# facebook/winterfell

Hardware: NVIDIA H100
Metric: prover_ms (lower is better)
Workload: dtype u64

## Files before the change

### winterfell_b200/csrc/minidft.cuh

```cuda
#pragma once
#include "gl64.cuh"

__device__ __forceinline__ void bf2(u64& a, u64& b) { gl_butterfly(a, b); }
template <int R>
__device__ __forceinline__ void mini_dft(u64* x);
template <>
__device__ __forceinline__ void mini_dft<1>(u64* x) { bf2(x[0], x[1]); }
template <>
__device__ __forceinline__ void mini_dft<2>(u64* x) {
    bf2(x[0], x[2]);
    bf2(x[1], x[3]);
    x[3] = gl_mul_2exp<48>(x[3]);
    bf2(x[0], x[1]);
    bf2(x[2], x[3]);
}
template <>
__device__ __forceinline__ void mini_dft<3>(u64* x);
template <>
__device__ __forceinline__ void mini_dft<3>(u64* x) {
    bf2(x[0], x[4]);
    bf2(x[1], x[5]);
    bf2(x[2], x[6]);
    bf2(x[3], x[7]);
    x[5] = gl_mul_2exp<24>(x[5]);
    x[6] = gl_mul_2exp<48>(x[6]);
    x[7] = gl_mul_2exp<72>(x[7]);
    mini_dft<2>(x);
    mini_dft<2>(x + 4);
}
template <>
__device__ __forceinline__ void mini_dft<4>(u64* x) {
    bf2(x[0], x[8]);
    bf2(x[1], x[9]);
    bf2(x[2], x[10]);
    bf2(x[3], x[11]);
    bf2(x[4], x[12]);
    bf2(x[5], x[13]);
    bf2(x[6], x[14]);
    bf2(x[7], x[15]);
    x[9] = gl_mul_2exp<12>(x[9]);
    x[10] = gl_mul_2exp<24>(x[10]);
    x[11] = gl_mul_2exp<36>(x[11]);
    x[12] = gl_mul_2exp<48>(x[12]);
    x[13] = gl_mul_2exp<60>(x[13]);
    x[14] = gl_mul_2exp<72>(x[14]);
    x[15] = gl_mul_2exp<84>(x[15]);
    mini_dft<3>(x);
    mini_dft<3>(x + 8);
}
template <>
__device__ __forceinline__ void mini_dft<5>(u64* x) {
#pragma unroll
    for (int q = 0; q < 16; q++) bf2(x[q], x[q + 16]);
    x[17] = gl_mul_2exp<6>(x[17]);
    x[18] = gl_mul_2exp<12>(x[18]);
    x[19] = gl_mul_2exp<18>(x[19]);
    x[20] = gl_mul_2exp<24>(x[20]);
    x[21] = gl_mul_2exp<30>(x[21]);
    x[22] = gl_mul_2exp<36>(x[22]);
    x[23] = gl_mul_2exp<42>(x[23]);
    x[24] = gl_mul_2exp<48>(x[24]);
    x[25] = gl_mul_2exp<54>(x[25]);
    x[26] = gl_mul_2exp<60>(x[26]);
    x[27] = gl_mul_2exp<66>(x[27]);
    x[28] = gl_mul_2exp<72>(x[28]);
    x[29] = gl_mul_2exp<78>(x[29]);
    x[30] = gl_mul_2exp<84>(x[30]);
    x[31] = gl_mul_2exp<90>(x[31]);
    mini_dft<4>(x);
    mini_dft<4>(x + 16);
}
__device__ __forceinline__ u32 brev(u32 v, int bits) { return __brev(v) >> (32 - bits); }

__device__ __forceinline__ u64 tw_lookup(const u64* tab, u32 e, u32 half) {
    u64 t = tab[e & (half - 1)];
    return (e & half) ? gl_neg(t) : t;
}
```

### winterfell_b200/csrc/ntt2.cu

```cuda
#include "minidft.cuh"
#include "ntt.cuh"

#ifndef NTT2_THREADS
#define NTT2_THREADS 256
#endif
#ifndef NTT2_MINB
#define NTT2_MINB 2
#endif
#define NTT2_TILE_ELEMS 8192

template <int LOGS>
struct Plan {
    static constexpr int rounds = LOGS >= 9 ? 3 : 2;
    static constexpr int r0 = (LOGS == 8) ? 4 : 3;
    static constexpr int r1 = (LOGS == 11 || LOGS == 8 || LOGS == 7) ? 4 : 3;
    static constexpr int r2 = LOGS >= 9 ? LOGS - r0 - r1 : 0;
    static_assert(LOGS >= 6 && LOGS <= 11, "plan covers 2^6 .. 2^11");
    static_assert(r0 + r1 + r2 == LOGS && (rounds == 2 || (r2 == 3 || r2 == 4)), "radices must add up");
    static constexpr int lanes = LOGS == 11 ? 4 : 8;
    static constexpr int tw0_entries = 1 << LOGS;
    static constexpr int tw1_entries = rounds == 3 ? (1 << (LOGS - r0)) : 0;
    static constexpr int tw_entries = tw0_entries + tw1_entries;
};
template <int LOGS> __host__ __device__ constexpr int plan_radix(int k) { return k == 0 ? Plan<LOGS>::r0 : (k == 1 ? Plan<LOGS>::r1 : Plan<LOGS>::r2); }
template <int LOGS> __host__ __device__ constexpr int plan_stage(int k) { return k == 0 ? 0 : (k == 1 ? Plan<LOGS>::r0 : Plan<LOGS>::r0 + Plan<LOGS>::r1); }

template <int LK>
__host__ __device__ constexpr u32 swz_const(u32 r) {
    u32 x = r >> LK, h = 0;
    while (x) { h ^= x & ((1u << LK) - 1); x >>= LK; }
    return h;
}
template <int LK>
__device__ __forceinline__ u32 swz_hash(u32 r) {
    if (LK == 1) return __popc(r >> 1) & 1;
    u32 x = r >> 2;
    x ^= x >> 4;
    x ^= x >> 8;
    x ^= x >> 2;
    return x & 3;
}
template <int LK>
__device__ __forceinline__ u32 prow(u32 r) { return r ^ swz_hash<LK>(r); }

__device__ __forceinline__ void bulk_init(u64* mbar, int tid) {
    if (tid == 0) {
        u32 mb = (u32)__cvta_generic_to_shared(mbar);
        asm volatile("mbarrier.init.shared::cta.b64 [%0], 1;" ::"r"(mb));
        asm volatile("fence.mbarrier_init.release.cluster;" ::: "memory");
    }
}
__device__ __forceinline__ void bulk_expect(u64* mbar, u32 bytes) {
    u32 mb = (u32)__cvta_generic_to_shared(mbar);
    asm volatile("mbarrier.arrive.expect_tx.shared::cta.b64 _, [%0], %1;" ::"r"(mb), "r"(bytes) : "memory");
}
__device__ __forceinline__ void bulk_copy(void* smem_dst, const void* gsrc, u32 bytes, u64* mbar) {
    u32 mb = (u32)__cvta_generic_to_shared(mbar), dst = (u32)__cvta_generic_to_shared(smem_dst);
    asm volatile("cp.async.bulk.shared::cluster.global.mbarrier::complete_tx::bytes [%0], [%1], %2, [%3];" ::"r"(dst), "l"(gsrc), "r"(bytes),
                 "r"(mb)
                 : "memory");
}
__device__ __forceinline__ void bulk_wait(u64* mbar) {
    u32 mb = (u32)__cvta_generic_to_shared(mbar), done = 0;
    while (!done)
        asm volatile("{\n\t.reg .pred p;\n\tmbarrier.try_wait.parity.shared::cta.b64 p, [%1], 0;\n\tselp.u32 %0, 1, 0, p;\n\t}" : "=r"(done) : "r"(mb) : "memory");
}

__device__ __forceinline__ void cp_async16(void* smem_dst, const void* gsrc, bool ok) {
    const u32 dst = (u32)__cvta_generic_to_shared(smem_dst);
    asm volatile("cp.async.cg.shared.global [%0], [%1], 16, %2;" ::"r"(dst), "l"(gsrc), "r"(ok ? 16 : 0) : "memory");
}
__device__ __forceinline__ void cp_async8(void* smem_dst, const void* gsrc, bool ok) {
    const u32 dst = (u32)__cvta_generic_to_shared(smem_dst);
    asm volatile("cp.async.ca.shared.global [%0], [%1], 8, %2;" ::"r"(dst), "l"(gsrc), "r"(ok ? 8 : 0) : "memory");
}
__device__ __forceinline__ void cp_async_commit() { asm volatile("cp.async.commit_group;" ::: "memory"); }
__device__ __forceinline__ void cp_async_wait_all() { asm volatile("cp.async.wait_group 0;" ::: "memory"); }

template <int LOGS, int K>
__device__ __forceinline__ void tile_round(u64* __restrict__ s, const u64* __restrict__ tw, const u64* __restrict__ pre, int tid) {
    constexpr int LANES = Plan<LOGS>::lanes, LK = LANES == 8 ? 1 : 2;
    constexpr int R = plan_radix<LOGS>(K), ST = plan_stage<LOGS>(K);
    constexpr int LOGSPAN = LOGS - ST - R;
    constexpr u32 SPAN = 1u << LOGSPAN;
    constexpr bool LAST = LOGSPAN == 0;
    constexpr u32 TASKS = (1u << LOGS) * LANES / 16;
    if (R == 4) {
        for (u32 task = tid; task < TASKS; task += NTT2_THREADS) {
            const u32 lane = task % LANES, bf = task / LANES;
            const u32 lo = bf & (SPAN - 1), base = ((bf >> LOGSPAN) << (LOGSPAN + 4)) + lo;
            const u32 hb = swz_hash<LK>(base);
            u64 x[16];
#pragma unroll
            for (int q = 0; q < 16; q++) {
                const u32 row = (base + ((u32)q << LOGSPAN)) ^ (hb ^ swz_const<LK>((u32)q << LOGSPAN));
                x[q] = s[row * LANES + lane];
            }
            if (K == 0 && pre) {
#pragma unroll
                for (int q = 0; q < 16; q++) x[q] = gl_mul(x[q], __ldg(pre + base + ((u32)q << LOGSPAN)));
            }
            mini_dft<4>(x);
            if (!LAST) {
                const ulonglong2* t2 = reinterpret_cast<const ulonglong2*>(tw + (size_t)lo * 16);
#pragma unroll
                for (int h = 0; h < 8; h++) {
                    const ulonglong2 w = t2[h];
                    if (h > 0) x[2 * h] = gl_mul(x[2 * h], w.x);
                    x[2 * h + 1] = gl_mul(x[2 * h + 1], w.y);
                }
            }
#pragma unroll
            for (int q = 0; q < 16; q++) {
                const u32 row = (base + ((u32)q << LOGSPAN)) ^ (hb ^ swz_const<LK>((u32)q << LOGSPAN));
                s[row * LANES + lane] = x[q];
            }
        }
    } else {
        constexpr int LP = LANES / 2;
        for (u32 task = tid; task < TASKS; task += NTT2_THREADS) {
            const u32 lp = task % LP, bf = task / LP;
            const u32 lo = bf & (SPAN - 1), base = ((bf >> LOGSPAN) << (LOGSPAN + 3)) + lo;
            const u32 hb = swz_hash<LK>(base);
            u64 xa[8], xb[8];
#pragma unroll
            for (int q = 0; q < 8; q++) {
                const u32 row = (base + ((u32)q << LOGSPAN)) ^ (hb ^ swz_const<LK>((u32)q << LOGSPAN));
                const ulonglong2 v = *reinterpret_cast<const ulonglong2*>(s + row * LANES + 2 * lp);
                xa[q] = v.x;
                xb[q] = v.y;
            }
            if (K == 0 && pre) {
#pragma unroll
                for (int q = 0; q < 8; q++) {
                    const u64 f = __ldg(pre + base + ((u32)q << LOGSPAN));
                    xa[q] = gl_mul(xa[q], f);
                    xb[q] = gl_mul(xb[q], f);
                }
            }
            mini_dft<3>(xa);
            mini_dft<3>(xb);
            if (!LAST) {
                const ulonglong2* t2 = reinterpret_cast<const ulonglong2*>(tw + (size_t)lo * 8);
#pragma unroll
                for (int h = 0; h < 4; h++) {
                    const ulonglong2 w = t2[h];
                    if (h > 0) { xa[2 * h] = gl_mul(xa[2 * h], w.x); xb[2 * h] = gl_mul(xb[2 * h], w.x); }
                    xa[2 * h + 1] = gl_mul(xa[2 * h + 1], w.y);
                    xb[2 * h + 1] = gl_mul(xb[2 * h + 1], w.y);
                }
            }
#pragma unroll
            for (int q = 0; q < 8; q++) {
                const u32 row = (base + ((u32)q << LOGSPAN)) ^ (hb ^ swz_const<LK>((u32)q << LOGSPAN));
                *reinterpret_cast<ulonglong2*>(s + row * LANES + 2 * lp) = make_ulonglong2(xa[q], xb[q]);
            }
        }
    }
}

template <int MODE, int LOGS>
__global__ void __launch_bounds__(NTT2_THREADS, NTT2_MINB) ntt2_pass_kernel(const NttPassParams p) {
    extern __shared__ __align__(16) u64 smem[];
    constexpr int LANES = Plan<LOGS>::lanes, LK = LANES == 8 ? 1 : 2, LP = LANES / 2;
    constexpr u32 S = 1u << LOGS;
    const int tid = threadIdx.x;
    const int W = p.W, logW = 31 - __clz(W);
    const int T = W >= LANES ? 1 : (LANES >> logW);
    const int chunks = W >= LANES ? W / LANES : 1;
    u64* s = smem;
    u64* rtw = s + (size_t)S * LANES;
    u64* ctw = rtw + Plan<LOGS>::tw_entries;
    u64* mbar = ctw + (p.has_post ? (size_t)S * T : 0);

    const bool ymap = p.y_in_out;
    const u32 tc = ymap ? blockIdx.y : blockIdx.x;
    const u32 tile = tc / chunks, q0 = (tc % chunks) * LANES;
    const u32 g = ymap ? blockIdx.z : blockIdx.y, b = ymap ? blockIdx.x : blockIdx.z;
    const u32 R = 1u << p.logR, C = 1u << p.logC;
    const u32 ncols = MODE == NTT_STRIDED ? C : R;

    {
        const u64* in = p.in + (size_t)g * p.in_seg_stride + (size_t)b * p.in_batch_stride;
        const u32 lp = tid % LP;
        const u32 l0 = 2 * lp;
        const u32 t0 = W >= LANES ? 0 : (l0 >> logW), t1 = W >= LANES ? 0 : ((l0 + 1) >> logW);
        const u32 w0 = W >= LANES ? q0 + l0 : (l0 & (W - 1)), w1 = W >= LANES ? q0 + l0 + 1 : ((l0 + 1) & (W - 1));
        const u32 c0 = tile * T + t0, c1 = tile * T + t1;
        const bool ok0 = c0 < ncols, ok1 = c1 < ncols;
        const bool yin = MODE == NTT_CONTIG && ymap;
        const u64 istride = MODE == NTT_STRIDED ? ((u64)W << p.logC) : (yin ? ((u64)p.out_row_mul << p.logR) * p.out_W : (u64)W);
        const u64* a0 = MODE == NTT_STRIDED ? in + (size_t)c0 * W + w0
                        : yin ? in + ((size_t)c0 * p.out_row_mul + (size_t)b * p.out_row_add) * p.out_W + p.out_col0 + w0
                              : in + (((size_t)c0 << p.logC) * W + w0);
        const u64* a1 = MODE == NTT_STRIDED ? in + (size_t)c1 * W + w1
                        : yin ? in + ((size_t)c1 * p.out_row_mul + (size_t)b * p.out_row_add) * p.out_W + p.out_col0 + w1
                              : in + (((size_t)c1 << p.logC) * W + w1);
        if (!ok0) a0 = p.in;
        if (!ok1) a1 = p.in;
        const u64 s0 = ok0 ? istride : 0, s1 = ok1 ? istride : 0;
        const bool vec = p.vec_in;
        constexpr u32 ROWS_PER_IT = NTT2_THREADS / LP;
#pragma unroll 4
        for (u32 i = tid / LP; i < S; i += ROWS_PER_IT) {
            u64* dst = s + prow<LK>(i) * LANES + l0;
            if (vec) {
                cp_async16(dst, a0 + i * s0, ok0);
            } else {
                cp_async8(dst, a0 + i * s0, ok0);
                cp_async8(dst + 1, a1 + i * s1, ok1);
            }
        }
        cp_async_commit();
    }

    bulk_init(mbar, tid);
    __syncthreads();
    if (tid == 0) {
        bulk_expect(mbar, Plan<LOGS>::tw_entries * 8);
        bulk_copy(rtw, p.sub_tw, Plan<LOGS>::tw_entries * 8, mbar);
    }

    if (p.has_post && T == 1) {
        const u32 M = 1u << p.logM, lo_mask = (1u << p.tw_split) - 1, c = tile;
        auto wpow = [&](u64 e64) {
            u32 e = (u32)(e64 & (M - 1));
            if (p.inverse && e) e = M - e;
            return gl_mul(p.tw_hi[e >> p.tw_split], p.tw_lo[e & lo_mask]);
        };
        u64 K = wpow((u64)(p.batch0 + b) * p.b_mul * c);
        if (p.ctab) K = gl_mul(K, p.ctab[c < ncols ? c : 0]);
        if (p.cconst != 1) K = gl_mul(K, p.cconst);
        const u64 step = wpow((u64)NTT2_THREADS * p.a_mul * c);
        u64 x = gl_mul(K, wpow((u64)tid * p.a_mul * c));
        for (u32 j = tid; j < S; j += NTT2_THREADS) {
            ctw[j] = x;
            x = gl_mul(x, step);
        }
    } else if (p.has_post) {
        const u32 M = 1u << p.logM, lo_mask = (1u << p.tw_split) - 1;
        for (u32 idx = tid; idx < S * (u32)T; idx += NTT2_THREADS) {
            const u32 j = idx / T, tt = idx % T, c = tile * T + tt;
            u64 e64 = ((u64)j * p.a_mul + (u64)(p.batch0 + b) * p.b_mul) * c;
            u32 e = (u32)(e64 & (M - 1));
            if (p.inverse && e) e = M - e;
            u64 x = gl_mul(p.tw_hi[e >> p.tw_split], p.tw_lo[e & lo_mask]);
            if (p.ctab) x = gl_mul(x, p.ctab[c < ncols ? c : 0]);
            if (p.cconst != 1) x = gl_mul(x, p.cconst);
            ctw[idx] = x;
        }
    }

    cp_async_wait_all();
    bulk_wait(mbar);
    __syncthreads();

    tile_round<LOGS, 0>(s, rtw, p.pre_tab ? p.pre_tab + (size_t)b * p.pre_batch_stride : nullptr, tid);
    __syncthreads();
    if (Plan<LOGS>::rounds == 3) {
        tile_round<LOGS, 1>(s, rtw + Plan<LOGS>::tw0_entries, nullptr, tid);
        __syncthreads();
        tile_round<LOGS, 2>(s, nullptr, nullptr, tid);
    } else {
        tile_round<LOGS, 1>(s, nullptr, nullptr, tid);
    }
    __syncthreads();

    u64* out = p.out + (size_t)g * p.out_seg_stride + (size_t)b * p.out_batch_stride;
    {
        const u32 lp = tid % LP, l0 = 2 * lp;
        const u32 t0 = W >= LANES ? 0 : (l0 >> logW), t1 = W >= LANES ? 0 : ((l0 + 1) >> logW);
        const u32 w0 = W >= LANES ? q0 + l0 : (l0 & (W - 1)), w1 = W >= LANES ? q0 + l0 + 1 : ((l0 + 1) & (W - 1));
        const u32 c0 = tile * T + t0, c1 = tile * T + t1;
        const bool ok0 = c0 < ncols, ok1 = c1 < ncols;
        u64 *o0, *o1, jstride;
        if (MODE == NTT_STRIDED && ymap) {
            o0 = out + (((size_t)c0 << p.logR) * p.out_row_mul + (size_t)b * p.out_row_add) * p.out_W + p.out_col0 + w0;
            o1 = out + (((size_t)c1 << p.logR) * p.out_row_mul + (size_t)b * p.out_row_add) * p.out_W + p.out_col0 + w1;
            jstride = (u64)p.out_row_mul * p.out_W;
        } else if (MODE == NTT_STRIDED) {
            o0 = out + (size_t)c0 * W + w0;
            o1 = out + (size_t)c1 * W + w1;
            jstride = (u64)W << p.logC;
        } else {
            o0 = out + ((size_t)c0 * p.out_row_mul + (size_t)b * p.out_row_add) * p.out_W + p.out_col0 + w0;
            o1 = out + ((size_t)c1 * p.out_row_mul + (size_t)b * p.out_row_add) * p.out_W + p.out_col0 + w1;
            jstride = ((u64)p.out_row_mul << p.logR) * p.out_W;
        }
        const bool post = p.has_post, scale = !p.has_post && p.cconst != 1, vec = p.vec_out;
        const u32 inv_mask = p.inverse ? (S - 1) : 0;
        constexpr u32 ROWS_PER_IT = NTT2_THREADS / LP;
#pragma unroll 4
        for (u32 j = tid / LP; j < S; j += ROWS_PER_IT) {
            const u32 jf = inv_mask ? ((S - j) & inv_mask) : j;
            const u32 r = __brev(jf) >> (32 - LOGS);
            ulonglong2 v = *reinterpret_cast<const ulonglong2*>(s + prow<LK>(r) * LANES + l0);
            if (post) {
                const u64 f0 = ctw[j * T + t0];
                v.x = gl_mul(v.x, f0);
                v.y = gl_mul(v.y, t1 == t0 ? f0 : ctw[j * T + t1]);
            } else if (scale) {
                v.x = gl_mul(v.x, p.cconst);
                v.y = gl_mul(v.y, p.cconst);
            }
            if (vec) {
                if (ok0) *reinterpret_cast<ulonglong2*>(o0 + (u64)j * jstride) = v;
            } else {
                if (ok0) o0[(u64)j * jstride] = v.x;
                if (ok1) o1[(u64)j * jstride] = v.y;
            }
        }
    }
}

template <int LOGS>
__global__ void ntt2_build_tw_kernel(u64* out, u64 w_s) {
    const u32 idx = blockIdx.x * blockDim.x + threadIdx.x;
    if (idx >= (u32)Plan<LOGS>::tw_entries) return;
    int k = idx < (u32)Plan<LOGS>::tw0_entries ? 0 : 1;
    const u32 li = k == 0 ? idx : idx - Plan<LOGS>::tw0_entries;
    const int r = plan_radix<LOGS>(k), st = plan_stage<LOGS>(k);
    const u32 lo = li >> r, qo = li & ((1u << r) - 1);
    const u32 e = (lo * (__brev(qo) >> (32 - r))) << st;
    out[idx] = gl_pow(w_s, e);
}

template <int LOGS>
static size_t smem_bytes_t(const NttPassParams& p) {
    const int lanes = Plan<LOGS>::lanes;
    const size_t S = (size_t)1 << LOGS, T = p.W >= lanes ? 1 : lanes / p.W;
    return (S * lanes + Plan<LOGS>::tw_entries + (p.has_post ? S * T : 0) + 2) * 8;
}
template <int MODE, int LOGS>
static cudaError_t launch_t(const NttPassParams& p, u32 n_segments, u32 n_batch, cudaStream_t st) {
    const int lanes = Plan<LOGS>::lanes;
    const u32 T = p.W >= lanes ? 1 : lanes / p.W, chunks = p.W >= lanes ? p.W / lanes : 1;
    const u32 ncols = MODE == NTT_STRIDED ? (1u << p.logC) : (1u << p.logR);
    const size_t smem = smem_bytes_t<LOGS>(p);
    const u32 tiles = ((ncols + T - 1) / T) * chunks;
    const dim3 grid = p.y_in_out ? dim3(n_batch, tiles, n_segments) : dim3(tiles, n_segments, n_batch);
    cudaError_t e = cudaFuncSetAttribute(ntt2_pass_kernel<MODE, LOGS>, cudaFuncAttributeMaxDynamicSharedMemorySize, (int)smem);
    if (e != cudaSuccess) return e;
    ntt2_pass_kernel<MODE, LOGS><<<grid, NTT2_THREADS, smem, st>>>(p);
    return cudaGetLastError();
}
template <int MODE>
static cudaError_t launch_m(const NttPassParams& p, u32 n_segments, u32 n_batch, cudaStream_t st) {
    switch (p.logS) {
        case 6: return launch_t<MODE, 6>(p, n_segments, n_batch, st);
        case 7: return launch_t<MODE, 7>(p, n_segments, n_batch, st);
        case 8: return launch_t<MODE, 8>(p, n_segments, n_batch, st);
        case 9: return launch_t<MODE, 9>(p, n_segments, n_batch, st);
        case 10: return launch_t<MODE, 10>(p, n_segments, n_batch, st);
        case 11: return launch_t<MODE, 11>(p, n_segments, n_batch, st);
    }
    return cudaErrorInvalidValue;
}
cudaError_t ntt2_launch_pass(int mode, const NttPassParams& p, u32 n_segments, u32 n_batch, cudaStream_t st) {
    return mode == NTT_STRIDED ? launch_m<NTT_STRIDED>(p, n_segments, n_batch, st) : launch_m<NTT_CONTIG>(p, n_segments, n_batch, st);
}
size_t ntt2_tw_entries(int logS) {
    switch (logS) {
        case 6: return Plan<6>::tw_entries; case 7: return Plan<7>::tw_entries; case 8: return Plan<8>::tw_entries;
        case 9: return Plan<9>::tw_entries; case 10: return Plan<10>::tw_entries; case 11: return Plan<11>::tw_entries;
    }
    return 0;
}
cudaError_t ntt2_build_tw(int logS, u64* d_out, cudaStream_t st) {
    const u64 w = gl_root_of_unity((u32)logS);
    const unsigned nb = (unsigned)((ntt2_tw_entries(logS) + 255) / 256);
    switch (logS) {
        case 6: ntt2_build_tw_kernel<6><<<nb, 256, 0, st>>>(d_out, w); break;
        case 7: ntt2_build_tw_kernel<7><<<nb, 256, 0, st>>>(d_out, w); break;
        case 8: ntt2_build_tw_kernel<8><<<nb, 256, 0, st>>>(d_out, w); break;
        case 9: ntt2_build_tw_kernel<9><<<nb, 256, 0, st>>>(d_out, w); break;
        case 10: ntt2_build_tw_kernel<10><<<nb, 256, 0, st>>>(d_out, w); break;
        case 11: ntt2_build_tw_kernel<11><<<nb, 256, 0, st>>>(d_out, w); break;
        default: return cudaErrorInvalidValue;
    }
    return cudaGetLastError();
}
```

Before: 115.4.

## Use radix-32 first round and shift-only twiddles for 2^11 tile NTT

For 2048-point tiles the plan becomes radix 32 then two radix-8 rounds. The middle twiddles between the two 64-point rounds are powers of the 64th root of unity, so they are applied as shift-based multiplications instead of table lookups and the second twiddle table is dropped. The radix-32 round uses a transposed twiddle table layout and precomputed smem row pointers, and the pre-multiply is done as a separate pass after the copy-in. Output indices are re-read from special registers to lower register pressure. The risk is more register pressure from holding 32 values per thread, plus branch divergence in the shift switch.

```diff
diff --git a/winterfell_b200/csrc/minidft.cuh b/winterfell_b200/csrc/minidft.cuh
--- a/winterfell_b200/csrc/minidft.cuh
+++ b/winterfell_b200/csrc/minidft.cuh
@@ -72,6 +72,22 @@
 }
 __device__ __forceinline__ u32 brev(u32 v, int bits) { return __brev(v) >> (32 - bits); }
 
+template <int E>
+__device__ __forceinline__ u64 gl_mul_w64(u64 x) {
+    constexpr int K = 3 * (E & 63);
+    if constexpr (K <= 96) return gl_mul_2exp<K>(x);
+    else return gl_neg(gl_mul_2exp<K - 96>(x));
+}
+template <int LO, int Q = 1>
+__device__ __forceinline__ void w64_layer(u64* xa, u64* xb) {
+    if constexpr (Q < 8) {
+        constexpr int E = LO * (((Q & 1) << 2) | (Q & 2) | ((Q >> 2) & 1));
+        xa[Q] = gl_mul_w64<E>(xa[Q]);
+        xb[Q] = gl_mul_w64<E>(xb[Q]);
+        w64_layer<LO, Q + 1>(xa, xb);
+    }
+}
+
 __device__ __forceinline__ u64 tw_lookup(const u64* tab, u32 e, u32 half) {
     u64 t = tab[e & (half - 1)];
     return (e & half) ? gl_neg(t) : t;
diff --git a/winterfell_b200/csrc/ntt2.cu b/winterfell_b200/csrc/ntt2.cu
--- a/winterfell_b200/csrc/ntt2.cu
+++ b/winterfell_b200/csrc/ntt2.cu
@@ -12,14 +12,16 @@
 template <int LOGS>
 struct Plan {
     static constexpr int rounds = LOGS >= 9 ? 3 : 2;
-    static constexpr int r0 = (LOGS == 8) ? 4 : 3;
-    static constexpr int r1 = (LOGS == 11 || LOGS == 8 || LOGS == 7) ? 4 : 3;
+    static constexpr int r0 = LOGS == 11 ? 5 : (LOGS == 8) ? 4 : 3;
+    static constexpr int r1 = (LOGS == 8 || LOGS == 7) ? 4 : 3;
     static constexpr int r2 = LOGS >= 9 ? LOGS - r0 - r1 : 0;
+    static constexpr bool shift1 = LOGS == 11;
     static_assert(LOGS >= 6 && LOGS <= 11, "plan covers 2^6 .. 2^11");
     static_assert(r0 + r1 + r2 == LOGS && (rounds == 2 || (r2 == 3 || r2 == 4)), "radices must add up");
+    static_assert(!shift1 || (rounds == 3 && r1 == 3 && r2 == 3), "the shift layer sits between two radix-8 rounds of 64 points");
     static constexpr int lanes = LOGS == 11 ? 4 : 8;
     static constexpr int tw0_entries = 1 << LOGS;
-    static constexpr int tw1_entries = rounds == 3 ? (1 << (LOGS - r0)) : 0;
+    static constexpr int tw1_entries = rounds == 3 && !shift1 ? (1 << (LOGS - r0)) : 0;
     static constexpr int tw_entries = tw0_entries + tw1_entries;
 };
 template <int LOGS> __host__ __device__ constexpr int plan_radix(int k) { return k == 0 ? Plan<LOGS>::r0 : (k == 1 ? Plan<LOGS>::r1 : Plan<LOGS>::r2); }
@@ -85,7 +87,35 @@
     constexpr u32 SPAN = 1u << LOGSPAN;
     constexpr bool LAST = LOGSPAN == 0;
     constexpr u32 TASKS = (1u << LOGS) * LANES / 16;
-    if (R == 4) {
+    if constexpr (R == 5) {
+        static_assert(!LAST, "a radix-32 round is followed by the 64-point rounds");
+        for (u32 task = tid; task < TASKS / 2; task += NTT2_THREADS) {
+            const u32 lane = task % LANES, bf = task / LANES;
+            const u32 lo = bf & (SPAN - 1), base = ((bf >> LOGSPAN) << (LOGSPAN + 5)) + lo;
+            static_assert((1 << LK) <= SPAN, "the row hash stays below the span");
+            const u32 hb = swz_hash<LK>(base);
+            u64* sp[1 << LK];
+#pragma unroll
+            for (int c = 0; c < (1 << LK); c++) sp[c] = s + (base ^ hb ^ (u32)c) * LANES + lane;
+            u64 x[32];
+#pragma unroll
+            for (int q = 0; q < 32; q++) x[q] = sp[swz_const<LK>((u32)q << LOGSPAN)][((u32)q << LOGSPAN) * LANES];
+            if (K == 0 && pre) {
+#pragma unroll
+                for (int q = 0; q < 32; q++) x[q] = gl_mul(x[q], __ldg(pre + base + ((u32)q << LOGSPAN)));
+            }
+            mini_dft<5>(x);
+            const ulonglong2* t2 = reinterpret_cast<const ulonglong2*>(tw) + lo;
+#pragma unroll
+            for (int h = 0; h < 16; h++) {
+                const ulonglong2 w = t2[h * SPAN];
+                if (h > 0) x[2 * h] = gl_mul(x[2 * h], w.x);
+                x[2 * h + 1] = gl_mul(x[2 * h + 1], w.y);
+#pragma unroll
+                for (int q = 2 * h; q < 2 * h + 2; q++) sp[swz_const<LK>((u32)q << LOGSPAN)][((u32)q << LOGSPAN) * LANES] = x[q];
+            }
+        }
+    } else if (R == 4) {
         for (u32 task = tid; task < TASKS; task += NTT2_THREADS) {
             const u32 lane = task % LANES, bf = task / LANES;
             const u32 lo = bf & (SPAN - 1), base = ((bf >> LOGSPAN) << (LOGSPAN + 4)) + lo;
@@ -118,8 +148,11 @@
         }
     } else {
         constexpr int LP = LANES / 2;
+        constexpr bool SHIFT = K == 1 && Plan<LOGS>::shift1;
+        static_assert(!SHIFT || (SPAN == 8 && LP == 2 && NTT2_THREADS % 256 == 0), "shift layer mapping");
         for (u32 task = tid; task < TASKS; task += NTT2_THREADS) {
-            const u32 lp = task % LP, bf = task / LP;
+            const u32 lp = task % LP;
+            const u32 bf = SHIFT ? ((((task >> 1) & 15) | ((task >> 8) << 4)) << 3) | ((task >> 5) & 7) : task / LP;
             const u32 lo = bf & (SPAN - 1), base = ((bf >> LOGSPAN) << (LOGSPAN + 3)) + lo;
             const u32 hb = swz_hash<LK>(base);
             u64 xa[8], xb[8];
@@ -140,7 +173,18 @@
             }
             mini_dft<3>(xa);
             mini_dft<3>(xb);
-            if (!LAST) {
+            if (SHIFT) {
+                switch (lo) {
+                    case 1: w64_layer<1>(xa, xb); break;
+                    case 2: w64_layer<2>(xa, xb); break;
+                    case 3: w64_layer<3>(xa, xb); break;
+                    case 4: w64_layer<4>(xa, xb); break;
+                    case 5: w64_layer<5>(xa, xb); break;
+                    case 6: w64_layer<6>(xa, xb); break;
+                    case 7: w64_layer<7>(xa, xb); break;
+                    default: break;
+                }
+            } else if (!LAST) {
                 const ulonglong2* t2 = reinterpret_cast<const ulonglong2*>(tw + (size_t)lo * 8);
 #pragma unroll
                 for (int h = 0; h < 4; h++) {
@@ -252,10 +296,21 @@
     }
 
     cp_async_wait_all();
+    const u64* pre = p.pre_tab ? p.pre_tab + (size_t)b * p.pre_batch_stride : nullptr;
+    constexpr bool PRE_APART = MODE == NTT_CONTIG && Plan<LOGS>::r0 == 5;
+    if (PRE_APART && pre) {
+        const u32 l0 = 2 * (tid % LP);
+        for (u32 i = tid / LP; i < S; i += NTT2_THREADS / LP) {
+            u64* d = s + prow<LK>(i) * LANES + l0;
+            const u64 f = __ldg(pre + i);
+            d[0] = gl_mul(d[0], f);
+            d[1] = gl_mul(d[1], f);
+        }
+    }
     bulk_wait(mbar);
     __syncthreads();
 
-    tile_round<LOGS, 0>(s, rtw, p.pre_tab ? p.pre_tab + (size_t)b * p.pre_batch_stride : nullptr, tid);
+    tile_round<LOGS, 0>(s, rtw, PRE_APART ? nullptr : pre, tid);
     __syncthreads();
     if (Plan<LOGS>::rounds == 3) {
         tile_round<LOGS, 1>(s, rtw + Plan<LOGS>::tw0_entries, nullptr, tid);
@@ -266,9 +321,17 @@
     }
     __syncthreads();
 
-    u64* out = p.out + (size_t)g * p.out_seg_stride + (size_t)b * p.out_batch_stride;
     {
-        const u32 lp = tid % LP, l0 = 2 * lp;
+        u32 wtid, bx, by, bz;
+        asm volatile("mov.u32 %0, %%tid.x;" : "=r"(wtid));
+        asm volatile("mov.u32 %0, %%ctaid.x;" : "=r"(bx));
+        asm volatile("mov.u32 %0, %%ctaid.y;" : "=r"(by));
+        asm volatile("mov.u32 %0, %%ctaid.z;" : "=r"(bz));
+        const u32 tc = ymap ? by : bx;
+        const u32 tile = tc / chunks, q0 = (tc % chunks) * LANES;
+        const u32 g = ymap ? bz : by, b = ymap ? bx : bz;
+        u64* out = p.out + (size_t)g * p.out_seg_stride + (size_t)b * p.out_batch_stride;
+        const u32 lp = wtid % LP, l0 = 2 * lp;
         const u32 t0 = W >= LANES ? 0 : (l0 >> logW), t1 = W >= LANES ? 0 : ((l0 + 1) >> logW);
         const u32 w0 = W >= LANES ? q0 + l0 : (l0 & (W - 1)), w1 = W >= LANES ? q0 + l0 + 1 : ((l0 + 1) & (W - 1));
         const u32 c0 = tile * T + t0, c1 = tile * T + t1;
@@ -291,7 +354,7 @@
         const u32 inv_mask = p.inverse ? (S - 1) : 0;
         constexpr u32 ROWS_PER_IT = NTT2_THREADS / LP;
 #pragma unroll 4
-        for (u32 j = tid / LP; j < S; j += ROWS_PER_IT) {
+        for (u32 j = wtid / LP; j < S; j += ROWS_PER_IT) {
             const u32 jf = inv_mask ? ((S - j) & inv_mask) : j;
             const u32 r = __brev(jf) >> (32 - LOGS);
             ulonglong2 v = *reinterpret_cast<const ulonglong2*>(s + prow<LK>(r) * LANES + l0);
@@ -320,7 +383,12 @@
     int k = idx < (u32)Plan<LOGS>::tw0_entries ? 0 : 1;
     const u32 li = k == 0 ? idx : idx - Plan<LOGS>::tw0_entries;
     const int r = plan_radix<LOGS>(k), st = plan_stage<LOGS>(k);
-    const u32 lo = li >> r, qo = li & ((1u << r) - 1);
+    u32 lo = li >> r, qo = li & ((1u << r) - 1);
+    if (r == 5) {
+        const u32 span = 1u << (LOGS - st - r);
+        lo = (li >> 1) & (span - 1);
+        qo = ((li >> 1) / span) * 2 + (li & 1);
+    }
     const u32 e = (lo * (__brev(qo) >> (32 - r))) << st;
     out[idx] = gl_pow(w_s, e);
 }
```

After: 113.3, median of 6. -1.8%, faster.
